# oscarkey/safe-exploration

Hardware: AMD Instinct MI355X
Metric: cem_particle_step_evals_per_s (higher is better)
Workload: dtype f64

## Files before the change

include/sx_amd.h:

```cpp
#ifndef SX_AMD_H
#define SX_AMD_H

#include <stdint.h>

#ifdef __cplusplus
extern "C" {
#endif

#define SX_MAX_NS 4
#define SX_MAX_NU 2
#define SX_MAX_D (SX_MAX_NS + SX_MAX_NU)
#define SX_MAX_M 16
#define SX_TILE 16

#define SX_OK 0
#define SX_ERR_ARG 1
#define SX_ERR_UNSUPPORTED 2
#define SX_ERR_LAUNCH 3

#define SX_STATUS_NAN 1
#define SX_STATUS_ZERO_FIX 2
#define SX_STATUS_UB_NONPOS 4

#define SX_OBJ_NEG_VARIANCE 0
// ... 79 lines not shown
    const double* net;
    const double* masks;
} sx_mlp_model;
int sx_mlp_predict(const sx_mlp_model* model, const double* z, int P, double* mean, double* var, double* jac, void* stream);
int sx_cem_rollout_mlp(const sx_mlp_model* model, const sx_env* env, int E, int P, int H, const double* x0, const double* q0,
                       const double* mean, const double* std, const double* noise, double* actions, double* traj,
                       double* sigma, double* obj_cost, double* con_cost, int32_t* status, void* stream);

int sx_cem_rollout_mlp_junk(const sx_mlp_model* model, const sx_env* env, int query_shift, int E, int P, int H,
                            const double* x0, const double* q0, const double* mean, const double* std, const double* noise,
                            double* actions, double* traj, double* sigma, double* obj_cost, double* con_cost,
                            int32_t* status, void* stream);

#define SX_PROF_ROLLOUT_FUSED 0
#define SX_PROF_RANK 1
#define SX_PROF_KSTAR_BIG 2
#define SX_PROF_TRMM_BIG 3
#define SX_PROF_STEP_BIG 4
#define SX_PROF_ROLLOUT_FEAT 5
#define SX_PROF_ROLLOUT_MLP 6
#define SX_PROF_KINDS 7
int sx_profile_enable(int max_launches);
int sx_profile_stride(int every);
int sx_profile_stride_kind(int kind, int every);
int sx_profile_collect(int kind, double* total_ms, int64_t* launches);
int sx_profile_disable(void);

#ifndef SX_WAVES
#define SX_WAVES 8
#endif

int sx_gp_pack_sizes(int n_s, int n_u, int n_train, int64_t* a_doubles, int64_t* tab_ints);

#define SX_STATUS_NOT_PD 8

int sx_gp_fit(const sx_gp_model* model, const double* y_train, double* work, double* linv, double* alpha,
              double* logdet, int32_t* status, void* stream);

int sx_gp_mll_grad(const sx_gp_model* model, const double* y_train, const double* linv, const double* alpha,
                   const double* logdet, double* work, double* mll, double* grad, void* stream);

int64_t sx_gp_append_workspace_bytes(int n_s, int n_train, int k);
int sx_gp_append(const sx_gp_model* model, int n_old, const double* y_train, const double* linv_old, const double* alpha_old,
                 const double* logdet_old, double* linv, double* alpha, double* logdet, int32_t* status,
                 void* workspace, int64_t workspace_bytes, void* stream);

#define SX_GP_FIT_ENTRY_BYTES 360
int64_t sx_gp_fit_table_bytes(int E);
int sx_gp_fit_table(const sx_gp_model* models, int E, const double* const* y_train, double* const* work,
                    double* const* linv, double* const* alpha, double* const* logdet, int32_t* status, double* mll,
                    double* grad, void* table);
int sx_gp_fit_multi(const sx_gp_model* models, int E, const void* table, void* stream);
int sx_gp_mll_grad_multi(const sx_gp_model* models, int E, const void* table, void* stream);

int64_t sx_gp_select_workspace_bytes(int n_s, int E, int n_max, int m);
int sx_gp_select(const sx_gp_model* models, int E, int m, const int32_t* seed_idx, int n_seed, int32_t* idx,
                 double* sel_var, int32_t* status, void* workspace, int64_t workspace_bytes, void* stream);

int sx_gp_pack(sx_gp_model* model, const double* linv, const double* alpha, void* stream);

int sx_gp_predict(const sx_gp_model* model, const double* z, int P, double* mean, double* var, double* jac,
                  void* workspace, int64_t workspace_bytes, void* stream);

int sx_gp_predict_var_jac(const sx_gp_model* model, const double* linv, const double* z, int P, double* jac_var,
                          void* stream);

// ... 226 lines not shown
```

safe_exploration_amd/_lib.py:

```python
import ctypes
import os
from ctypes import POINTER, Structure, c_char_p, c_double, c_int, c_int32, c_int64, c_uint8, c_void_p

import numpy as np
import torch

SX_MAX_NS = 4
SX_MAX_NU = 2
SX_MAX_D = SX_MAX_NS + SX_MAX_NU
SX_MAX_M = 16
SX_SAT_MAX_DIM = SX_MAX_NS + 1
SX_TILE = 16
SX_GP_FIT_ENTRY_BYTES = 360
SX_FEAT_MAX_WIDTH = 32
SX_FEAT_MAX_LAYERS = 3
SX_MLP_MAX_HIDDEN = 4
SX_MLP_MAX_WIDTH = 64

SX_OK, SX_ERR_ARG, SX_ERR_UNSUPPORTED, SX_ERR_LAUNCH = 0, 1, 2, 3
SX_STATUS_NAN, SX_STATUS_ZERO_FIX, SX_STATUS_UB_NONPOS, SX_STATUS_NOT_PD = 1, 2, 4, 8
SX_OBJ_NEG_VARIANCE, SX_OBJ_AFFINE_ABS = 0, 1
SX_CON_TERMINAL, SX_CON_ALL_STATES = 0, 1
SX_PROF_ROLLOUT_FUSED, SX_PROF_RANK, SX_PROF_KSTAR_BIG, SX_PROF_TRMM_BIG, SX_PROF_STEP_BIG, SX_PROF_ROLLOUT_FEAT, SX_PROF_ROLLOUT_MLP = range(7)
PROF_KERNELS = {SX_PROF_ROLLOUT_FUSED: 'cem_rollout_kernel', SX_PROF_RANK: 'cem_rank_kernel',
# ... 20 lines not shown
                ('net', c_void_p), ('wbar', c_void_p), ('minv', c_void_p)]


class SxMlpModel(Structure):
    _fields_ = [('n_s', c_int32), ('n_u', c_int32), ('n_hidden', c_int32), ('n_out', c_int32), ('n_samples', c_int32),
                ('predict_std', c_int32), ('width', c_int32 * (SX_MLP_MAX_HIDDEN + 1)), ('net', c_void_p),
                ('masks', c_void_p)]


class SxEnv(Structure):
    _fields_ = [('n_s', c_int32), ('n_u', c_int32), ('m', c_int32), ('obj_mode', c_int32), ('con_mode', c_int32),
                ('reserved', c_int32), ('beta', c_double),
                ('a', c_double * (SX_MAX_NS * SX_MAX_NS)), ('b', c_double * (SX_MAX_NS * SX_MAX_NU)),
                ('k_fb', c_double * (SX_MAX_NU * SX_MAX_NS)), ('l_mu', c_double * SX_MAX_NS),
                ('l_sigma', c_double * SX_MAX_NS), ('h_mat', c_double * (SX_MAX_M * SX_MAX_NS)),
                ('h_vec', c_double * SX_MAX_M), ('u_min', c_double * SX_MAX_NU), ('u_max', c_double * SX_MAX_NU),
                ('obj_w_abs', c_double * SX_MAX_NS), ('obj_target', c_double * SX_MAX_NS),
                ('obj_w_lin', c_double * SX_MAX_NS)]


class SxSatCost(Structure):
    _fields_ = [('trig_idx', c_int32), ('rank', c_int32), ('target', c_double * SX_SAT_MAX_DIM),
                ('v', c_double * (SX_SAT_MAX_DIM * SX_SAT_MAX_DIM))]


class SxConSet(Structure):
    _fields_ = [('m_obs', c_int32), ('ctrl_ellipsoid', c_int32), ('h_mat_obs', c_double * (SX_MAX_M * SX_MAX_NS)),
                ('h_obs', c_double * SX_MAX_M)]


SIGNATURES = {
    'sx_version': (c_char_p, []),
    'sx_gp_pack_sizes': (c_int, [c_int, c_int, c_int, POINTER(c_int64), POINTER(c_int64)]),
    'sx_gp_fit': (c_int, [POINTER(SxGpModel)] + [c_void_p] * 7),
    'sx_gp_mll_grad': (c_int, [POINTER(SxGpModel)] + [c_void_p] * 8),
    'sx_gp_append_workspace_bytes': (c_int64, [c_int, c_int, c_int]),
    'sx_gp_append': (c_int, [POINTER(SxGpModel), c_int] + [c_void_p] * 9 + [c_int64, c_void_p]),
    'sx_gp_fit_table_bytes': (c_int64, [c_int]),
    'sx_gp_fit_table': (c_int, [POINTER(SxGpModel), c_int] + [POINTER(c_void_p)] * 5 + [c_void_p] * 4),
    'sx_gp_fit_multi': (c_int, [POINTER(SxGpModel), c_int, c_void_p, c_void_p]),
    'sx_gp_mll_grad_multi': (c_int, [POINTER(SxGpModel), c_int, c_void_p, c_void_p]),
    'sx_gp_select_workspace_bytes': (c_int64, [c_int, c_int, c_int, c_int]),
    'sx_gp_select': (c_int, [POINTER(SxGpModel), c_int, c_int, c_void_p, c_int, c_void_p, c_void_p, c_void_p, c_void_p,
                             c_int64, c_void_p]),
    'sx_gp_pack': (c_int, [POINTER(SxGpModel), c_void_p, c_void_p, c_void_p]),
    'sx_gp_predict': (c_int, [POINTER(SxGpModel), c_void_p, c_int, c_void_p, c_void_p, c_void_p, c_void_p, c_int64,
                              c_void_p]),
    'sx_gp_predict_workspace_bytes': (c_int64, [POINTER(SxGpModel), c_int]),
    'sx_gp_predict_var_jac': (c_int, [POINTER(SxGpModel), c_void_p, c_void_p, c_int, c_void_p, c_void_p]),
    'sx_gp_predict_mean_hessian': (c_int, [POINTER(SxGpModel), c_void_p, c_void_p, c_int, c_void_p, c_void_p]),
    'sx_feat_features': (c_int, [POINTER(SxFeatModel), c_void_p, c_int, c_void_p, c_void_p]),
    'sx_feat_fit': (c_int, [POINTER(SxFeatModel), c_void_p, c_void_p, c_int, POINTER(c_double)] + [c_void_p] * 5),
    'sx_feat_predict': (c_int, [POINTER(SxFeatModel), c_void_p, c_int, c_void_p, c_void_p, c_void_p, c_void_p]),
    'sx_cem_rollout_feat': (c_int, [POINTER(SxFeatModel), POINTER(SxEnv), c_int, c_int, c_int] + [c_void_p] * 12),
    'sx_mlp_predict': (c_int, [POINTER(SxMlpModel), c_void_p, c_int, c_void_p, c_void_p, c_void_p, c_void_p]),
    'sx_cem_rollout_mlp': (c_int, [POINTER(SxMlpModel), POINTER(SxEnv), c_int, c_int, c_int] + [c_void_p] * 12),
    'sx_cem_rollout_feat_junk': (c_int, [POINTER(SxFeatModel), POINTER(SxEnv), c_int, c_int, c_int, c_int] + [c_void_p] * 12),
    'sx_cem_rollout_mlp_junk': (c_int, [POINTER(SxMlpModel), POINTER(SxEnv), c_int, c_int, c_int, c_int] + [c_void_p] * 12),
    'sx_onestep_reach': (c_int, [POINTER(SxEnv), c_int] + [c_void_p] * 11),
    'sx_polytope_distance': (c_int, [POINTER(SxEnv), c_int, c_void_p, c_void_p, c_double, c_void_p, c_void_p,
                                     c_void_p]),
    'sx_cem_rollout': (c_int, [POINTER(SxGpModel), POINTER(SxEnv), c_int, c_int, c_int] + [c_void_p] * 12
                       + [c_int64, c_void_p]),
    'sx_cem_rollout_elites': (c_int, [POINTER(SxGpModel), POINTER(SxEnv), c_int, c_int, c_int, c_void_p, c_void_p, c_void_p,
                                      c_int] + [c_void_p] * 10),
    'sx_cem_rollout_junk': (c_int, [POINTER(SxGpModel), POINTER(SxEnv), c_int, c_int, c_int, c_int] + [c_void_p] * 12
# ... 156 lines not shown
```

safe_exploration_amd/csrc/sx_big.hpp:

```cpp
#pragma once
#include <hip/hip_runtime.h>

#include "sx_gp.hpp"
#include "sx_reach.hpp"
#include "sx_step.hpp"

namespace sx {

constexpr int kBigTile = 128;
constexpr int kBigRb = kBigTile / 16;
constexpr int kBigThreads = 256;

struct BigWs {
    double* ks;
    double* part;
    double* mj;
    double* zs;
    double* pst;
    double* qst;
    int64_t total;
};

inline BigWs big_ws_layout(double* base, int ns, int d_in, int n_pad, int64_t particles) {
    const int64_t p128 = (particles + kBigTile - 1) / kBigTile * kBigTile;
// ... 211 lines not shown
#pragma unroll
                for (int n = 0; n < NT; ++n) {
                    acc[m][n] = __builtin_amdgcn_mfma_f64_16x16x4f64(a[m].x, b[n].x, acc[m][n], 0, 0, 0);
                    acc[m][n] = __builtin_amdgcn_mfma_f64_16x16x4f64(a[m].y, b[n].y, acc[m][n], 0, 0, 0);
                }
            }
        }
    };

#pragma unroll
    for (int c = 0; c < NBUF - 1; ++c)
        if (c < nchunks) issue_chunk(c, c);
    auto step = [&](int c, auto bufc) {
        constexpr int BUF = decltype(bufc)::value;
        const int younger = (nchunks - 1 - c) < (NBUF - 2) ? (nchunks - 1 - c) : (NBUF - 2);
        if (younger >= 1 && NBUF >= 3) {
            if (is_k)
                asm volatile("s_waitcnt vmcnt(%0)" ::"n"(kPiecesK) : "memory");
            else
                asm volatile("s_waitcnt vmcnt(%0)" ::"n"(kPiecesW) : "memory");
        } else
            asm volatile("s_waitcnt vmcnt(0)" ::: "memory");
        __builtin_amdgcn_s_barrier();
        asm volatile("" ::: "memory");
        if (c + NBUF - 1 < nchunks) issue_chunk(c + NBUF - 1, (BUF + NBUF - 1) % NBUF);
        compute(c, BUF);
    };
    static_assert(NBUF == 2 || NBUF == 3, "the wait counts are written for one or two chunks in flight");
    for (int c = 0; c < nchunks; c += NBUF) {
        step(c, std::integral_constant<int, 0>{});
        if (c + 1 < nchunks) step(c + 1, std::integral_constant<int, 1>{});
        if (NBUF == 3 && c + 2 < nchunks) step(c + 2, std::integral_constant<int, 2 % NBUF>{});
    }
#pragma unroll
    for (int n = 0; n < NT; ++n) {
        const int64_t p = ((int64_t)pg * PT + NT * wc + n) * 16 + (lane & 15);
        double s = 0.0;
#pragma unroll
        for (int m = 0; m < 4; ++m) {
            const int row0 = (rb0 + 4 * wr + m) * 16 + (lane >> 4);
#pragma unroll
            for (int r = 0; r < 4; ++r) {
                const int row = row0 + 4 * r;
                const double v = acc[m][n][r];
                if (row < gc.n_train)
                    s = fma(v, v, s);
                else if (row - gc.n_train <= D)
                    ws.mj[((int64_t)d * (D + 1) + (row - gc.n_train)) * p128 + p] = v;
            }
        }
        s += __shfl_xor(s, 16);
        s += __shfl_xor(s, 32);
        if (lane < 16) ws.part[((int64_t)d * row_tiles * 2 + rt * 2 + wr) * p128 + p] = s;
    }
  }
}

struct BigStep {
    const double* actions;
    double* traj;
    double* sigma;
    double* obj;
    double* con;
    int* status;
    int H, t, row_parts;
    int have_q;
};

template <int NS, int NU>
__global__ void step_big_kernel(GpConst<NS, NS + NU> gc, ReachConst<NS, NU> rc, CostConst<SX_MAX_M, NS, NU> cc,
                                BigStep bs, BigWs ws, int64_t total, int64_t p128) {
    constexpr int D = NS + NU;
    const int64_t g = blockIdx.x * (int64_t)blockDim.x + threadIdx.x;
    if (g >= total) return;
    double p[NS], Q[NS][NS], z[D], u[NU], mean[NS], var[NS], jac[NS][D], p1[NS], Q1[NS][NS];
#pragma unroll
    for (int i = 0; i < NS; ++i) {
        p[i] = ws.pst[g * NS + i];
#pragma unroll
        for (int j = 0; j < NS; ++j) Q[i][j] = ws.qst[(g * NS + i) * NS + j];
// ... 51 lines not shown
```

safe_exploration_amd/csrc/sx_fit.hpp:

```cpp
#pragma once
#include <hip/hip_runtime.h>

#include "../../include/sx_amd.h"
#include "sx_gp.hpp"
#include "sx_reach.hpp"

namespace sx {

template <int MAXNS, int MAXD>
struct PackArgs {
    double inv_ls2[MAXNS * MAXD];
};

__global__ void pack_a_kernel(const double* __restrict__ linv, const double* __restrict__ alpha,
                              const double* __restrict__ x_train, PackArgs<SX_MAX_NS, SX_MAX_D> args, int n_s, int D, int n,
                              int n_pad, double* __restrict__ a_pack) {
    const int nrb = n_pad >> 4;
    const int64_t wpo = w_pairs_per_output(nrb);
    const int64_t total = (int64_t)n_s * wpo * 128;
    for (int64_t i = blockIdx.x * (int64_t)blockDim.x + threadIdx.x; i < total; i += (int64_t)gridDim.x * blockDim.x) {
        const int slot = (int)(i & 1);
        const int lane = (int)((i >> 1) & 63);
        int64_t pair = i >> 7;
        const int d = (int)(pair / wpo);
        pair -= (int64_t)d * wpo;
        int rb = (int)((sqrt(4.0 * (double)pair + 1.0) - 1.0) * 0.5);
        while ((int64_t)rb * (rb + 1) > pair) --rb;
        while ((int64_t)(rb + 1) * (rb + 2) <= pair) ++rb;
        const int q = (int)(pair - (int64_t)rb * (rb + 1));
        const int row = rb * 16 + (lane & 15);
        const int k = 8 * q + 4 * slot + (lane >> 4);
        double v = 0.0;
        if (row < n) {
            if (k <= row) v = linv[((int64_t)d * n + row) * n + k];
        } else if (row - n <= D && k < n) {
            const int r = row - n;
            const double al = alpha[(int64_t)d * n + k];
            v = (r == 0) ? al : al * x_train[(int64_t)k * D + r - 1] * args.inv_ls2[d * D + r - 1];
        }
        a_pack[i] = v;
    }
}

constexpr int kFitThreads = 1024;
constexpr int kFitMaxN = 4096;

struct FitArgs {
    double inv_ls2[SX_MAX_NS * SX_MAX_D];
    double outputscale[SX_MAX_NS];
    double noise[SX_MAX_NS];
    const double* x;
    const double* y;
    double* lmat;
    double* linv;
    double* alpha;
    double* logdet;
    int* status;
    int n, D, n_s, panel_cols;
};

struct GpFitEntry {
    double inv_ls2[SX_MAX_NS * SX_MAX_D];
    double outputscale[SX_MAX_NS];
    double noise[SX_MAX_NS];
    const double* x;
    const double* y;
// ... 363 lines not shown
```

safe_exploration_amd/csrc/sx_gp.hpp:

```cpp
#pragma once
#include <hip/hip_runtime.h>
#include <type_traits>
#include "../../include/sx_amd.h"

namespace sx {

typedef double v4d __attribute__((ext_vector_type(4)));
typedef double v2d __attribute__((ext_vector_type(2)));

__host__ __device__ inline int64_t w_pairs_per_output(int nrb) { return (int64_t)nrb * (nrb + 1); }
__host__ __device__ inline int64_t w_pack_doubles(int n_s, int n_pad) {
    return (int64_t)n_s * w_pairs_per_output(n_pad / 16) * 128;
}
__host__ __device__ inline int64_t a_pack_doubles(int n_s, int n_pad) { return w_pack_doubles(n_s, n_pad); }
__host__ __device__ inline int gp_n_pad(int n_train, int d_in) { return (n_train + 1 + d_in + 15) / 16 * 16; }

__device__ __forceinline__ int frag_index(int c, int k) {
    return (((k >> 3) * 64 + ((k & 3) << 4) + c) << 1) + ((k >> 2) & 1);
}

template <class A>
__device__ __forceinline__ double gp_kernel_value(const A& a, int d, int D, int i, int j) {
    double q = 0.0;
    for (int c = 0; c < D; ++c) {
        const double df = a.x[(size_t)i * D + c] - a.x[(size_t)j * D + c];
        q += df * df * a.inv_ls2[d * D + c];
    }
    return a.outputscale[d] * exp(-0.5 * q);
}

constexpr int kExpTab = 256;
__device__ const double kExp2Tab[kExpTab] = {
    1.0, 1.0027112750502025, 1.0054299011128027, 1.0081558981184175,
    1.0108892860517005, 1.0136300849514894, 1.016378314910953, 1.019133996077738,
    1.0218971486541166, 1.0246677928971357, 1.0274459491187637, 1.030231637686041,
    1.0330248790212284, 1.0358256936019572, 1.0386341019613787, 1.041450124688316,
    1.0442737824274138, 1.0471050958792898, 1.0499440858006872, 1.0527907730046264,
    1.0556451783605572, 1.0585073227945128, 1.061377227289262, 1.0642549128844645,
    1.0671404006768237, 1.0700337118202419, 1.0729348675259756, 1.075843889062791,
    1.0787607977571199, 1.0816856149932152, 1.0846183622133092, 1.0875590609177697,
    1.0905077326652577, 1.0934643990728858, 1.0964290818163769, 1.099401802630222,
    1.102382583307841, 1.1053714457017412, 1.1083684117236787, 1.1113735033448175,
    1.1143867425958924, 1.1174081515673693, 1.1204377524096067, 1.12347556733302,
    1.1265216186082418, 1.129575928566288, 1.1326385195987192, 1.1357094141578055,
    1.1387886347566916, 1.1418762039695616, 1.1449721444318042, 1.148076478840179,
    1.1511892299529827, 1.154310420590216, 1.1574400736337511, 1.1605782120274988,
    1.1637248587775775, 1.1668800369524817, 1.1700437696832502, 1.1732160801636373,
    1.1763969916502812, 1.1795865274628758, 1.182784710984341, 1.1859915656609938,
// ... 371 lines not shown
    auto issue = [&](MfmaStage& st, int i) {
        st.z = head.z[i];
        st.w = head.w[i];
        st.a0 = head.a[i][0];
        st.a1 = head.a[i][1];
        const v2d* b = kbase + head.y[i];
        st.b0 = b[0];
        st.b1 = b[64 * NSL];
    };

    v4d acc = {0.0, 0.0, 0.0, 0.0};
    auto step = [&](const MfmaStage& cur, MfmaStage& nx, int inext) {
        acc = __builtin_amdgcn_mfma_f64_16x16x4f64(cur.a0.x, cur.b0.x, acc, 0, 0, 0);
        SX_PIN();
        decode_a(nx);
        nx.a0 = load_a(0);
        SX_PIN();
        acc = __builtin_amdgcn_mfma_f64_16x16x4f64(cur.a0.y, cur.b0.y, acc, 0, 0, 0);
        SX_PIN();
        nx.a1 = load_a(1024);
        decode_b(inext);
        SX_PIN();
        acc = __builtin_amdgcn_mfma_f64_16x16x4f64(cur.a1.x, cur.b1.x, acc, 0, 0, 0);
        SX_PIN();
        nx.b0 = bp[0];
        nx.b1 = bp[64 * NSL];
        SX_PIN();
        acc = __builtin_amdgcn_mfma_f64_16x16x4f64(cur.a1.y, cur.b1.y, acc, 0, 0, 0);
        SX_PIN();
        if (__builtin_expect(cur.w & kStageLast, 0)) {
            const int d = cur.z & 255;
            double s;
            if (cur.w & kStageExtra) {
                const int row0 = (cur.z >> 8) * 16 + (lane >> 4);
                s = 0.0;
#pragma unroll
                for (int r = 0; r < 4; ++r) {
                    const int row = row0 + 4 * r;
                    if (row < gc.n_train)
                        s = fma(acc[r], acc[r], s);
                    else if (row - gc.n_train <= D)
                        lds.mj[d * 256 + (row - gc.n_train) * 16 + (lane & 15)] = acc[r];
                }
            } else {
                s = fma(acc[3], acc[3], fma(acc[2], acc[2], fma(acc[1], acc[1], acc[0] * acc[0])));
            }
#pragma unroll
            for (int dd = 0; dd < NS; ++dd) ssq[dd] = fma(s, (d == dd) ? 1.0 : 0.0, ssq[dd]);
            acc = v4d{0.0, 0.0, 0.0, 0.0};
        }
    };

    if (nst > 0) {
        MfmaStage s0, s1, s2, s3;
        issue(s0, 0);
        issue(s1, 1);
        issue(s2, 2);
        int i = 0;
        for (; i + 4 <= nst; i += 4) {
            step(s0, s3, i + 3);
            step(s1, s0, i + 4);
            step(s2, s1, i + 5);
            step(s3, s2, i + 6);
        }
        if (i < nst) {
            step(s0, s3, i + 3);
            if (i + 1 < nst) {
                step(s1, s0, i + 4);
                if (i + 2 < nst) step(s2, s1, i + 5);
            }
        }
    }
#pragma unroll
    for (int d = 0; d < NS; ++d) {
// ... 26 lines not shown
```

safe_exploration_amd/csrc/sx_gp_fit.hip:

```cpp
#include <hip/hip_runtime.h>

#include <algorithm>
#include <cstring>

#include "../../include/sx_amd.h"
#include "sx_fit.hpp"
#include "sx_fit_blocked.hpp"
#include "sx_host.hpp"
#include "sx_launch.hpp"

namespace sx {

static bool gp_shape_ok(int n_s, int n_u, int n_train, bool wide) {
    if (n_s <= 0 || n_s > SX_MAX_NS || n_u <= 0 || n_train <= 0) return false;
    return n_u <= (wide ? SX_MAX_D - n_s : SX_MAX_NU);
}
static bool gp_shape_ok(const sx_gp_model& m, bool wide) { return gp_shape_ok(m.n_s, m.n_u, m.n_train, wide); }

static int fit_panel_cols(int n) {
    const size_t lds_budget = 112 * 1024;
    const int nb = (int)(lds_budget / (sizeof(double) * (size_t)n));
    return nb > 32 ? 32 : (nb < 1 ? 1 : nb);
}
static_assert(kBlockedFitMinN * 32 * sizeof(double) < 64 * 1024, "gp_fit_kernel's panel must stay below 64 KB of LDS");
// ... 29 lines not shown
    for (int e = 0; e < E; ++e)
        if (models[e].n_s != ns || models[e].n_u != nu || models[e].n_train <= 0 || !models[e].x_train) return SX_ERR_ARG;
    for (int e = 0; e < E; ++e)
        if (models[e].n_train > kFitMaxN) return SX_ERR_UNSUPPORTED;
    return SX_OK;
}

struct FitMultiPlan {
    int nb_max = 0, small_n_max = 0, n_max = 0;
};
static FitMultiPlan plan_fit_multi(const sx_gp_model* models, int E) {
    FitMultiPlan plan;
    for (int e = 0; e < E; ++e) {
        const int n = models[e].n_train;
        plan.n_max = std::max(plan.n_max, n);
        if (n > kBlockedFitMinN)
            plan.nb_max = std::max(plan.nb_max, blocks_of(n));
        else
            plan.small_n_max = std::max(plan.small_n_max, n);
    }
    return plan;
}

}

extern "C" {

int sx_gp_pack_sizes(int n_s, int n_u, int n_train, int64_t* a_doubles, int64_t* tab_ints) {
    if (!sx::gp_shape_ok(n_s, n_u, n_train, true)) return SX_ERR_ARG;
    const int n_pad = sx::gp_n_pad(n_train, n_s + n_u);
    if (a_doubles) *a_doubles = sx::a_pack_doubles(n_s, n_pad);
    if (tab_ints) *tab_ints = sx::gp_stage_tab_ints(n_s, n_pad, SX_WAVES);
    return SX_OK;
}

int sx_gp_fit(const sx_gp_model* model, const double* y_train, double* work, double* linv, double* alpha,
              double* logdet, int32_t* status, void* stream) {
    if (!model || !model->x_train || !y_train || !work || !linv || !alpha || !logdet || !status) return SX_ERR_ARG;
    if (!sx::gp_shape_ok(*model, true)) return SX_ERR_ARG;
    if (model->n_train > sx::kFitMaxN) return SX_ERR_UNSUPPORTED;
    auto fill = [&](auto& a) {
        std::memset(&a, 0, sizeof(a));
        sx::copy_hyper(*model, a.inv_ls2, a.outputscale, a.noise);
        a.x = model->x_train;
        a.y = y_train;
        a.lmat = work;
        a.linv = linv;
        a.alpha = alpha;
        a.logdet = logdet;
        a.status = status;
        a.n = model->n_train;
        a.D = model->n_s + model->n_u;
        a.n_s = model->n_s;
    };
    if (model->n_train > sx::kBlockedFitMinN) {
        sx::BlockedFitArgs ba;
        fill(ba);
        ba.nblk = sx::blocks_of(ba.n);
        sx::launch_blocked_fit<false>(ba, ba.nblk, ba.n_s, sizeof(double) * (size_t)ba.n, (hipStream_t)stream);
        return sx::check_launch();
    }
    sx::FitArgs fa;
    fill(fa);
    fa.panel_cols = sx::fit_panel_cols(fa.n);
    const size_t lds = sizeof(double) * (size_t)fa.n * fa.panel_cols;
    hipLaunchKernelGGL(sx::gp_fit_kernel<false>, dim3(model->n_s), dim3(sx::kFitThreads), lds, (hipStream_t)stream, fa);
// ... 170 lines not shown
```

safe_exploration_amd/csrc/sx_rollout_rh.hpp:

```cpp
#pragma once
#include <hip/hip_runtime.h>

#include "../../include/sx_amd.h"
#include "sx_rollout_rw.hpp"

#ifndef SX_RH_REGP
#define SX_RH_REGP 26
#endif
#ifndef SX_RH_LEAD
#define SX_RH_LEAD -1
#endif
#ifndef SX_RH_LDSP
#define SX_RH_LDSP 8
#endif
#ifndef SX_RH_PFG
#define SX_RH_PFG 6
#endif
#ifndef SX_RH_PFL
#define SX_RH_PFL 2
#endif
#ifndef SX_RH_RBMAJOR
#define SX_RH_RBMAJOR 1
#endif
#ifndef SX_RH_PRIO
// ... 178 lines not shown
            }
        }
        while (done < npend) {
            ops[n++] = RhOp{kRhRowEpi, 0, pend_rb[done], 0, pend_d[done], 0};
            ++done;
        }
        const RhPlan<NS, NRB> plan{};
        for (int d = 0; d < NS; ++d)
            if (plan.has(WAVE, d)) ops[n++] = RhOp{kRhFinalEpi, 0, 0, 0, d, 0};
    }
};

template <int NS, int D, int NRB, int WAVE, int REGP, int LDSP>
__device__ __forceinline__ void rh_mfma_phase(const GpConst<NS, D>& gc, GpTileLds<NS, D>& lds, const v2d* wlds_wave, int lane,
                                              const v2d (&wreg)[REGP]) {
    constexpr int PF = SX_RW_PF, PFL = SX_RH_PFL, PFG = SX_RH_PFG;
    constexpr int MAXP = RhPlan<NS, NRB>{}.max_pairs();
    static constexpr RhProgram<NS, NRB, WAVE, REGP, LDSP, PF, PFL, PFG> prog{};
    static constexpr RhStream<NS, NRB, MAXP, REGP, LDSP> stream{};
    const v2d* kbase = reinterpret_cast<const v2d*>(lds.kfrag) + lane;
    typedef const __attribute__((address_space(1))) v2d* gv2d;
    typedef const __attribute__((address_space(3))) v2d* lv2d;
    const v2d* ap_opaque = reinterpret_cast<const v2d*>(gc.a_pack) + lane;
    asm volatile("" : "+v"(ap_opaque));
    const gv2d ap = (gv2d)ap_opaque;
    const lv2d wl_base = (lv2d)wlds_wave + lane;
    v4d acc[NRB];
    v2d b[PF + 1];
    v2d wl[PFL + 1];
    v2d wg[PFG + 1];
    double ssq[NS];
#pragma unroll
    for (int d = 0; d < NS; ++d) ssq[d] = 0.0;
    static_for<0, prog.n>([&](auto ktag) {
        constexpr RhOp op = prog.ops[decltype(ktag)::value];
        if constexpr (op.kind == kRhLoadB) {
            b[op.slot] = kbase[(op.q * NS + op.d) * 64];
        } else if constexpr (op.kind == kRhLoadWL) {
            wl[op.i % (PFL + 1)] = wl_base[(op.i - REGP) * 64];
        } else if constexpr (op.kind == kRhLoadWG) {
            wg[op.i % (PFG + 1)] = ap[(size_t)stream.pair[WAVE][op.i] * 64];
        } else if constexpr (op.kind == kRhMfma) {
#if SX_RH_PRIO == 2
            if constexpr ((4 * op.e) / prog.total != (4 * (op.e - 1)) / prog.total || op.e == 0)
                __builtin_amdgcn_s_setprio(3 - (4 * op.e) / prog.total);
#endif
            SX_PIN();
            const v2d bq = b[op.slot];
            v2d a;
            if constexpr (op.i < REGP)
                a = wreg[op.i];
            else if constexpr (op.i < REGP + LDSP)
                a = wl[op.i % (PFL + 1)];
            else
                a = wg[op.i % (PFG + 1)];
            if constexpr (op.q == 0)
                acc[op.rb] = __builtin_amdgcn_mfma_f64_16x16x4f64(a.x, bq.x, v4d{0.0, 0.0, 0.0, 0.0}, 0, 0, 0);
            else
                acc[op.rb] = __builtin_amdgcn_mfma_f64_16x16x4f64(a.x, bq.x, acc[op.rb], 0, 0, 0);
            acc[op.rb] = __builtin_amdgcn_mfma_f64_16x16x4f64(a.y, bq.y, acc[op.rb], 0, 0, 0);
            SX_PIN();
        } else if constexpr (op.kind == kRhRowEpi) {
            constexpr int rb = op.rb, d = op.d;
            double s;
            if constexpr (rb >= NRB - 2) {
                const int row0 = rb * 16 + (lane >> 4);
                s = 0.0;
#pragma unroll
                for (int r = 0; r < 4; ++r) {
                    const int row = row0 + 4 * r;
                    if (row < gc.n_train)
                        s = fma(acc[rb][r], acc[rb][r], s);
                    else if (row - gc.n_train <= D)
                        lds.mj[d * 256 + (row - gc.n_train) * 16 + (lane & 15)] = acc[rb][r];
                }
            } else {
                s = fma(acc[rb][3], acc[rb][3], fma(acc[rb][2], acc[rb][2], fma(acc[rb][1], acc[rb][1], acc[rb][0] * acc[rb][0])));
            }
            ssq[d] += s;
        } else {
            constexpr int d = op.d;
            const v4d tot = __builtin_amdgcn_mfma_f64_16x16x4f64(1.0, ssq[d], v4d{0.0, 0.0, 0.0, 0.0}, 0, 0, 0);
            if (lane < 16) lds.part[(WAVE * NS + d) * 16 + lane] = tot[0];
        }
    });
}

template <int NS, int D, int NRB, bool WITH_JAC, typename G>
__device__ __forceinline__ void rh_collect(const G& gc, const GpTileLds<NS, D>& lds, int c, const double (&z)[D],
                                           double (&mean)[NS], double (&var)[NS], double (&jac)[NS][D]) {
    constexpr RhPlan<NS, NRB> plan{};
#pragma unroll
    for (int d = 0; d < NS; ++d) {
        double q = 0.0;
#pragma unroll
        for (int w = 0; w < kRhWaves; ++w)
            if (plan.has(w, d)) q += lds.part[(w * NS + d) * 16 + c];
        var[d] = (gc.outputscale[d] - q) + gc.noise[d];
        const double m = lds.mj[d * 256 + c];
        mean[d] = m;
        if constexpr (WITH_JAC) {
#pragma unroll
            for (int j = 0; j < D; ++j) jac[d][j] = lds.mj[d * 256 + (1 + j) * 16 + c] - z[j] * gc.inv_ls2[d * D + j] * m;
        }
    }
}
// ... 476 lines not shown
```

safe_exploration_amd/csrc/sx_rollout_rw.hpp:

```cpp
#pragma once
#include <hip/hip_runtime.h>

#include "../../include/sx_amd.h"
#include "sx_exp2_tab2048.hpp"
#include "sx_gp.hpp"
#include "sx_reach.hpp"
#include "sx_refit.hpp"
#include "sx_rollout.hpp"
#include "sx_rw_launch.hpp"

#ifndef SX_RW_LDSCONST
#define SX_RW_LDSCONST 1
#endif
#ifndef SX_RW_POLYLANES
#define SX_RW_POLYLANES 1
#endif
#ifndef SX_RW_PF
#define SX_RW_PF 2
#endif
#ifndef SX_RW_RCLOCAL
#define SX_RW_RCLOCAL 0
#endif
#ifndef SX_RW_POLYFOLD
#define SX_RW_POLYFOLD 0
// ... 50 lines not shown
};

template <int NS, int NRB>
constexpr bool rw_fits() {
    return RwPlan<NS, NRB>{}.max_pairs() <= kRwMaxPairs;
}

template <int NS, int NRB, int MAXP>
struct RwLoadTab {
    int pair[kRwWaves][MAXP];
    constexpr RwLoadTab() : pair{} {
        const RwPlan<NS, NRB> plan{};
        constexpr int wpo = NRB * (NRB + 1);
        for (int w = 0; w < kRwWaves; ++w) {
            int idx = 0;
            for (int d = 0; d < NS; ++d)
                for (int rb = NRB - 1; rb >= 0; --rb) {
                    if (plan.wave_of[d][rb] != w) continue;
                    for (int q = 0; q < 2 * (rb + 1); ++q) pair[w][idx++] = d * wpo + rb * (rb + 1) + q;
                }
            for (; idx < MAXP; ++idx) pair[w][idx] = 0;
        }
    }
};

template <int NS, int D, int NRB, int MAXP>
__device__ __forceinline__ void rw_load_w(const GpConst<NS, D>& gc, int wave, int lane, v2d (&wreg)[MAXP]) {
    static constexpr RwLoadTab<NS, NRB, MAXP> tab{};
    const v2d* __restrict__ ap = reinterpret_cast<const v2d*>(gc.a_pack) + lane;
#pragma unroll
    for (int i = 0; i < MAXP; ++i) wreg[i] = ap[(size_t)tab.pair[wave][i] * 64];
}

template <int NS, int D, int NRB, int WAVE, int MAXP, int PF = SX_RW_PF>
__device__ __forceinline__ void rw_mfma_phase(const GpConst<NS, D>& gc, GpTileLds<NS, D>& lds, int lane,
                                              const v2d (&wreg)[MAXP]) {
    constexpr RwPlan<NS, NRB> plan{};
    const v2d* kbase = reinterpret_cast<const v2d*>(lds.kfrag) + lane;
    int first[NS][NRB];
    {
        int idx = 0;
#pragma unroll
        for (int d = 0; d < NS; ++d)
#pragma unroll
            for (int rb = NRB - 1; rb >= 0; --rb) {
                first[d][rb] = idx;
                if (plan.wave_of[d][rb] == WAVE) idx += 2 * (rb + 1);
            }
    }
    static_for<0, NS>([&](auto dtag) {
        constexpr int d = decltype(dtag)::value;
        constexpr int qmax = plan.qmax(WAVE, d);
        if constexpr (qmax > 0) {
        v4d acc[NRB];
        v2d b[PF + 1];
#pragma unroll
        for (int q = 0; q < PF && q < qmax; ++q) b[q] = kbase[(q * NS + d) * 64];
#pragma unroll
        for (int q = 0; q < qmax; ++q) {
            if (q + PF < qmax) b[(q + PF) % (PF + 1)] = kbase[((q + PF) * NS + d) * 64];
            SX_PIN();
            const v2d bq = b[q % (PF + 1)];
#pragma unroll
            for (int rb = NRB - 1; rb >= 0; --rb) {
                if (plan.wave_of[d][rb] != WAVE || q >= 2 * (rb + 1)) continue;
                const v2d a = wreg[first[d][rb] + q];
                if (q == 0)
                    acc[rb] = __builtin_amdgcn_mfma_f64_16x16x4f64(a.x, bq.x, v4d{0.0, 0.0, 0.0, 0.0}, 0, 0, 0);
                else
                    acc[rb] = __builtin_amdgcn_mfma_f64_16x16x4f64(a.x, bq.x, acc[rb], 0, 0, 0);
                acc[rb] = __builtin_amdgcn_mfma_f64_16x16x4f64(a.y, bq.y, acc[rb], 0, 0, 0);
            }
            SX_PIN();
        }
        double ssq = 0.0;
#pragma unroll
        for (int rb = NRB - 1; rb >= 0; --rb) {
            if (plan.wave_of[d][rb] != WAVE) continue;
            double s;
            if (rb >= NRB - 2) {
                const int row0 = rb * 16 + (lane >> 4);
                s = 0.0;
#pragma unroll
                for (int r = 0; r < 4; ++r) {
                    const int row = row0 + 4 * r;
                    if (row < gc.n_train)
                        s = fma(acc[rb][r], acc[rb][r], s);
                    else if (row - gc.n_train <= D)
                        lds.mj[d * 256 + (row - gc.n_train) * 16 + (lane & 15)] = acc[rb][r];
                }
            } else {
                s = fma(acc[rb][3], acc[rb][3], fma(acc[rb][2], acc[rb][2], fma(acc[rb][1], acc[rb][1], acc[rb][0] * acc[rb][0])));
            }
            ssq += s;
        }
        const v4d tot = __builtin_amdgcn_mfma_f64_16x16x4f64(1.0, ssq, v4d{0.0, 0.0, 0.0, 0.0}, 0, 0, 0);
        if (lane < 16) lds.part[(WAVE * NS + d) * 16 + lane] = tot[0];
        }
    });
}

constexpr double kExpScale2 = 2048.0 / 0.693147180559945309417232;
constexpr double kExpUnit2 = 0.693147180559945309417232 / 2048.0;

template <int NS, int D>
struct RwKstarLds {
    double* rows;
    double* tab;
    double* xbar;
    static __host__ __device__ size_t doubles(int n_pad) { return (size_t)n_pad * (D + NS) + (n_pad & 1) + kExpTab2 + 2 + ((D + 1) & ~1); }
    __device__ void carve(double* base, int n_pad) {
        rows = base;
        tab = rows + (size_t)n_pad * (D + NS) + (n_pad & 1);
        xbar = tab + kExpTab2 + 2;
    }
};

template <int NS, int D>
__device__ __forceinline__ void rw_kstar_setup(const GpConst<NS, D>& gc, const RwKstarLds<NS, D>& kl, double* kfrag) {
    const int tid = threadIdx.x, lane = tid & 63;
    double xb[D];
// ... 540 lines not shown
```

Baseline: 465.3 million.

## Shift packed GP rows to skip zero K-chunks in rollout MFMA loops

Moves the padding rows of the packed triangular Linv/A layout into the top of the first row block, so the triangular structure leaves whole 4-wide K chunks all zero. The rollout MFMA loops then skip those chunks behind runtime scalar-uniform checks on the shift and n_train cap. This cuts the f64 MFMA count in the hot rollout path. In exchange it adds scalar branches, a position-to-row remap in every epilogue, and a hard-coded opt-out for one shape (NS=2, D=3, NRB=13).

New measurement: 468.9 million, median of 6. No clear change (+0.8%).

```diff
diff --git a/include/sx_amd.h b/include/sx_amd.h
--- a/include/sx_amd.h
+++ b/include/sx_amd.h
@@ -135,6 +135,9 @@
 
 int sx_gp_pack_sizes(int n_s, int n_u, int n_train, int64_t* a_doubles, int64_t* tab_ints);
 
+int sx_gp_row_shift(int n_train, int d_in);
+int sx_gp_block_chunks(int n_train, int d_in, int rb);
+
 #define SX_STATUS_NOT_PD 8
 
 int sx_gp_fit(const sx_gp_model* model, const double* y_train, double* work, double* linv, double* alpha,
diff --git a/safe_exploration_amd/_lib.py b/safe_exploration_amd/_lib.py
--- a/safe_exploration_amd/_lib.py
+++ b/safe_exploration_amd/_lib.py
@@ -76,6 +76,8 @@
 SIGNATURES = {
     'sx_version': (c_char_p, []),
     'sx_gp_pack_sizes': (c_int, [c_int, c_int, c_int, POINTER(c_int64), POINTER(c_int64)]),
+    'sx_gp_row_shift': (c_int, [c_int, c_int]),
+    'sx_gp_block_chunks': (c_int, [c_int, c_int, c_int]),
     'sx_gp_fit': (c_int, [POINTER(SxGpModel)] + [c_void_p] * 7),
     'sx_gp_mll_grad': (c_int, [POINTER(SxGpModel)] + [c_void_p] * 8),
     'sx_gp_append_workspace_bytes': (c_int64, [c_int, c_int, c_int]),
diff --git a/safe_exploration_amd/csrc/sx_big.hpp b/safe_exploration_amd/csrc/sx_big.hpp
--- a/safe_exploration_amd/csrc/sx_big.hpp
+++ b/safe_exploration_amd/csrc/sx_big.hpp
@@ -267,20 +267,22 @@
         if (c + 1 < nchunks) step(c + 1, std::integral_constant<int, 1>{});
         if (NBUF == 3 && c + 2 < nchunks) step(c + 2, std::integral_constant<int, 2 % NBUF>{});
     }
+    const int shift = gp_row_shift(gc.n_train, D);
 #pragma unroll
     for (int n = 0; n < NT; ++n) {
         const int64_t p = ((int64_t)pg * PT + NT * wc + n) * 16 + (lane & 15);
         double s = 0.0;
 #pragma unroll
         for (int m = 0; m < 4; ++m) {
-            const int row0 = (rb0 + 4 * wr + m) * 16 + (lane >> 4);
+            const int pos0 = (rb0 + 4 * wr + m) * 16 + (lane >> 4);
 #pragma unroll
             for (int r = 0; r < 4; ++r) {
-                const int row = row0 + 4 * r;
+                const int row = gp_pos_row(pos0 + 4 * r, shift, gc.n_train, D);
                 const double v = acc[m][n][r];
+                if (row < 0) continue;
                 if (row < gc.n_train)
                     s = fma(v, v, s);
-                else if (row - gc.n_train <= D)
+                else
                     ws.mj[((int64_t)d * (D + 1) + (row - gc.n_train)) * p128 + p] = v;
             }
         }
diff --git a/safe_exploration_amd/csrc/sx_fit.hpp b/safe_exploration_amd/csrc/sx_fit.hpp
--- a/safe_exploration_amd/csrc/sx_fit.hpp
+++ b/safe_exploration_amd/csrc/sx_fit.hpp
@@ -28,10 +28,11 @@
         while ((int64_t)rb * (rb + 1) > pair) --rb;
         while ((int64_t)(rb + 1) * (rb + 2) <= pair) ++rb;
         const int q = (int)(pair - (int64_t)rb * (rb + 1));
-        const int row = rb * 16 + (lane & 15);
+        const int row = gp_pos_row(rb * 16 + (lane & 15), gp_row_shift(n, D), n, D);
         const int k = 8 * q + 4 * slot + (lane >> 4);
         double v = 0.0;
-        if (row < n) {
+        if (row < 0) {
+        } else if (row < n) {
             if (k <= row) v = linv[((int64_t)d * n + row) * n + k];
         } else if (row - n <= D && k < n) {
             const int r = row - n;
diff --git a/safe_exploration_amd/csrc/sx_gp.hpp b/safe_exploration_amd/csrc/sx_gp.hpp
--- a/safe_exploration_amd/csrc/sx_gp.hpp
+++ b/safe_exploration_amd/csrc/sx_gp.hpp
@@ -14,6 +14,39 @@
 }
 __host__ __device__ inline int64_t a_pack_doubles(int n_s, int n_pad) { return w_pack_doubles(n_s, n_pad); }
 __host__ __device__ inline int gp_n_pad(int n_train, int d_in) { return (n_train + 1 + d_in + 15) / 16 * 16; }
+__host__ __device__ inline int gp_row_shift(int n_train, int d_in) {
+    return (gp_n_pad(n_train, d_in) - (n_train + 1 + d_in)) & ~3;
+}
+__host__ __device__ inline int gp_pos_row(int p, int s, int n_train, int d_in) {
+    const int row = p < 16 ? (p < 16 - s ? p : -1) : p - s;
+    return row > n_train + d_in ? -1 : row;
+}
+__host__ __device__ inline int gp_block_chunks(int n_train, int d_in, int rb) {
+    const int own = 4 * (rb + 1) - gp_row_shift(n_train, d_in) / 4, cap = (n_train + 3) / 4;
+    return own < cap ? own : cap;
+}
+template <int D, int NRB>
+__device__ __forceinline__ bool gp_chunk_needed(int rb, int c, int s4, int cap) {
+    static_assert(D <= 11, "see the bounds above");
+#ifdef SX_NO_CHUNK_SKIP
+    return true;
+#endif
+#ifdef SX_CHUNK_FIXED_S4
+    s4 = SX_CHUNK_FIXED_S4;
+    cap = SX_CHUNK_FIXED_CAP;
+    if (rb < NRB - 1) return s4 < 4 * (rb + 1) - c;
+    return c < cap;
+#endif
+    if (rb < NRB - 1) {
+        const int m = 4 * (rb + 1) - c;
+        if (m > 3) return true;
+        asm volatile("" : "+s"(s4));
+        return s4 < m;
+    }
+    if (c == 0 || c < 4 * NRB - (D + 16) / 4) return true;
+    asm volatile("" : "+s"(cap));
+    return c < cap;
+}
 
 __device__ __forceinline__ int frag_index(int c, int k) {
     return (((k >> 3) * 64 + ((k & 3) << 4) + c) << 1) + ((k >> 2) & 1);
@@ -451,14 +484,16 @@
             const int d = cur.z & 255;
             double s;
             if (cur.w & kStageExtra) {
-                const int row0 = (cur.z >> 8) * 16 + (lane >> 4);
+                const int pos0 = (cur.z >> 8) * 16 + (lane >> 4);
+                const int shift = gp_row_shift(gc.n_train, D);
                 s = 0.0;
 #pragma unroll
                 for (int r = 0; r < 4; ++r) {
-                    const int row = row0 + 4 * r;
+                    const int row = gp_pos_row(pos0 + 4 * r, shift, gc.n_train, D);
+                    if (row < 0) continue;
                     if (row < gc.n_train)
                         s = fma(acc[r], acc[r], s);
-                    else if (row - gc.n_train <= D)
+                    else
                         lds.mj[d * 256 + (row - gc.n_train) * 16 + (lane & 15)] = acc[r];
                 }
             } else {
diff --git a/safe_exploration_amd/csrc/sx_gp_fit.hip b/safe_exploration_amd/csrc/sx_gp_fit.hip
--- a/safe_exploration_amd/csrc/sx_gp_fit.hip
+++ b/safe_exploration_amd/csrc/sx_gp_fit.hip
@@ -85,6 +85,16 @@
     if (a_doubles) *a_doubles = sx::a_pack_doubles(n_s, n_pad);
     if (tab_ints) *tab_ints = sx::gp_stage_tab_ints(n_s, n_pad, SX_WAVES);
     return SX_OK;
+}
+
+int sx_gp_row_shift(int n_train, int d_in) {
+    if (n_train < 1 || d_in < 1 || d_in > SX_MAX_D) return -1;
+    return sx::gp_row_shift(n_train, d_in);
+}
+
+int sx_gp_block_chunks(int n_train, int d_in, int rb) {
+    if (n_train < 1 || d_in < 1 || d_in > SX_MAX_D || rb < 0 || rb >= sx::gp_n_pad(n_train, d_in) / 16) return -1;
+    return sx::gp_block_chunks(n_train, d_in, rb);
 }
 
 int sx_gp_fit(const sx_gp_model* model, const double* y_train, double* work, double* linv, double* alpha,
diff --git a/safe_exploration_amd/csrc/sx_rollout_rh.hpp b/safe_exploration_amd/csrc/sx_rollout_rh.hpp
--- a/safe_exploration_amd/csrc/sx_rollout_rh.hpp
+++ b/safe_exploration_amd/csrc/sx_rollout_rh.hpp
@@ -234,6 +234,7 @@
     double ssq[NS];
 #pragma unroll
     for (int d = 0; d < NS; ++d) ssq[d] = 0.0;
+    const int shift = gp_row_shift(gc.n_train, D), s4 = shift >> 2, cap = (gc.n_train + 3) >> 2;
     static_for<0, prog.n>([&](auto ktag) {
         constexpr RhOp op = prog.ops[decltype(ktag)::value];
         if constexpr (op.kind == kRhLoadB) {
@@ -256,24 +257,29 @@
                 a = wl[op.i % (PFL + 1)];
             else
                 a = wg[op.i % (PFG + 1)];
-            if constexpr (op.q == 0)
+            if constexpr (op.q == 0) {
                 acc[op.rb] = __builtin_amdgcn_mfma_f64_16x16x4f64(a.x, bq.x, v4d{0.0, 0.0, 0.0, 0.0}, 0, 0, 0);
-            else
+                if (gp_chunk_needed<D, NRB>(op.rb, 1, s4, cap))
+                    acc[op.rb] = __builtin_amdgcn_mfma_f64_16x16x4f64(a.y, bq.y, acc[op.rb], 0, 0, 0);
+            } else if (gp_chunk_needed<D, NRB>(op.rb, 2 * op.q, s4, cap)) {
                 acc[op.rb] = __builtin_amdgcn_mfma_f64_16x16x4f64(a.x, bq.x, acc[op.rb], 0, 0, 0);
-            acc[op.rb] = __builtin_amdgcn_mfma_f64_16x16x4f64(a.y, bq.y, acc[op.rb], 0, 0, 0);
+                if (gp_chunk_needed<D, NRB>(op.rb, 2 * op.q + 1, s4, cap))
+                    acc[op.rb] = __builtin_amdgcn_mfma_f64_16x16x4f64(a.y, bq.y, acc[op.rb], 0, 0, 0);
+            }
             SX_PIN();
         } else if constexpr (op.kind == kRhRowEpi) {
             constexpr int rb = op.rb, d = op.d;
             double s;
             if constexpr (rb >= NRB - 2) {
-                const int row0 = rb * 16 + (lane >> 4);
+                const int pos0 = rb * 16 + (lane >> 4);
                 s = 0.0;
 #pragma unroll
                 for (int r = 0; r < 4; ++r) {
-                    const int row = row0 + 4 * r;
+                    const int row = gp_pos_row(pos0 + 4 * r, shift, gc.n_train, D);
+                    if (row < 0) continue;
                     if (row < gc.n_train)
                         s = fma(acc[rb][r], acc[rb][r], s);
-                    else if (row - gc.n_train <= D)
+                    else
                         lds.mj[d * 256 + (row - gc.n_train) * 16 + (lane & 15)] = acc[rb][r];
                 }
             } else {
diff --git a/safe_exploration_amd/csrc/sx_rollout_rw.hpp b/safe_exploration_amd/csrc/sx_rollout_rw.hpp
--- a/safe_exploration_amd/csrc/sx_rollout_rw.hpp
+++ b/safe_exploration_amd/csrc/sx_rollout_rw.hpp
@@ -106,11 +106,18 @@
     for (int i = 0; i < MAXP; ++i) wreg[i] = ap[(size_t)tab.pair[wave][i] * 64];
 }
 
+template <int NS, int D, int NRB>
+constexpr bool rw_skips_chunks() {
+    return !(NS == 2 && D == 3 && NRB == 13);
+}
+
 template <int NS, int D, int NRB, int WAVE, int MAXP, int PF = SX_RW_PF>
 __device__ __forceinline__ void rw_mfma_phase(const GpConst<NS, D>& gc, GpTileLds<NS, D>& lds, int lane,
                                               const v2d (&wreg)[MAXP]) {
     constexpr RwPlan<NS, NRB> plan{};
+    constexpr bool SKIP = rw_skips_chunks<NS, D, NRB>();
     const v2d* kbase = reinterpret_cast<const v2d*>(lds.kfrag) + lane;
+    const int shift = gp_row_shift(gc.n_train, D), s4 = shift >> 2, cap = (gc.n_train + 3) >> 2;
     int first[NS][NRB];
     {
         int idx = 0;
@@ -139,11 +146,15 @@
             for (int rb = NRB - 1; rb >= 0; --rb) {
                 if (plan.wave_of[d][rb] != WAVE || q >= 2 * (rb + 1)) continue;
                 const v2d a = wreg[first[d][rb] + q];
-                if (q == 0)
+                if (q == 0) {
                     acc[rb] = __builtin_amdgcn_mfma_f64_16x16x4f64(a.x, bq.x, v4d{0.0, 0.0, 0.0, 0.0}, 0, 0, 0);
-                else
+                    if (!SKIP || gp_chunk_needed<D, NRB>(rb, 1, s4, cap))
+                        acc[rb] = __builtin_amdgcn_mfma_f64_16x16x4f64(a.y, bq.y, acc[rb], 0, 0, 0);
+                } else if (!SKIP || gp_chunk_needed<D, NRB>(rb, 2 * q, s4, cap)) {
                     acc[rb] = __builtin_amdgcn_mfma_f64_16x16x4f64(a.x, bq.x, acc[rb], 0, 0, 0);
-                acc[rb] = __builtin_amdgcn_mfma_f64_16x16x4f64(a.y, bq.y, acc[rb], 0, 0, 0);
+                    if (!SKIP || gp_chunk_needed<D, NRB>(rb, 2 * q + 1, s4, cap))
+                        acc[rb] = __builtin_amdgcn_mfma_f64_16x16x4f64(a.y, bq.y, acc[rb], 0, 0, 0);
+                }
             }
             SX_PIN();
         }
@@ -153,14 +164,15 @@
             if (plan.wave_of[d][rb] != WAVE) continue;
             double s;
             if (rb >= NRB - 2) {
-                const int row0 = rb * 16 + (lane >> 4);
+                const int pos0 = rb * 16 + (lane >> 4);
                 s = 0.0;
 #pragma unroll
                 for (int r = 0; r < 4; ++r) {
-                    const int row = row0 + 4 * r;
+                    const int row = gp_pos_row(pos0 + 4 * r, shift, gc.n_train, D);
+                    if (row < 0) continue;
                     if (row < gc.n_train)
                         s = fma(acc[rb][r], acc[rb][r], s);
-                    else if (row - gc.n_train <= D)
+                    else
                         lds.mj[d * 256 + (row - gc.n_train) * 16 + (lane & 15)] = acc[rb][r];
                 }
             } else {
```
